# AntreasAntoniou/HowToTrainYourMAMLPytorch

Measured on NVIDIA H100. Metric: meta-tasks/sec (5-way, 5 inner steps, second order), higher is better.
Workload: dtype fp32

## Files before the change

### howtotrainyourmamlpytorch_b200/csrc/engine.cu

```cuda
#include <cstdio>
#include <cstdlib>
#include <cstring>
#include <cmath>
#include <string>
#include <vector>

#include "../../include/maml_b200.h"
#include "common.cuh"
#include "tc_common.cuh"

static thread_local std::string g_err;
static int fail(const std::string& m) { g_err = m; return 1; }

#define CK(call) do { cudaError_t e__ = (call); if (e__ != cudaSuccess) { \
  return fail(std::string(#call) + ": " + cudaGetErrorString(e__)); } } while (0)

static inline long long rup(long long x, long long m) { return (x + m - 1) / m * m; }

struct Profiler {
  struct Rec { int cat; double flops; cudaEvent_t a, b; };
  std::vector<Rec> recs;
  std::vector<cudaEvent_t> pool;
  size_t used = 0;
  cudaEvent_t get() {
// ... 115 lines not shown
static thread_local LaunchContext g_launch_ctx{&g_default_options, false, nullptr, nullptr};
const LaunchContext& launch_ctx() { return g_launch_ctx; }

struct LaunchScope {
  LaunchContext saved;
  explicit LaunchScope(maml_b200_handle* h) : LaunchScope(h, false, nullptr) {}
  LaunchScope(maml_b200_handle* h, cudaStream_t main) : LaunchScope(h, h->pdl, main) {}
  ~LaunchScope() { g_launch_ctx = saved; }
 private:
  LaunchScope(maml_b200_handle* h, bool pdl, cudaStream_t main) : saved(g_launch_ctx) {
    g_launch_ctx = LaunchContext{&h->opt, pdl, main, h->profiling ? &h->prof : nullptr};
  }
};

int num_sms() {
  static int n = 0;
  if (n == 0) {
    int dev = 0;
    if (cudaGetDevice(&dev) != cudaSuccess || cudaDeviceGetAttribute(&n, cudaDevAttrMultiProcessorCount, dev) != cudaSuccess || n <= 0) n = 132;
  }
  return n;
}

extern "C" int maml_b200_abi_version(void) { return MAML_B200_ABI_VERSION; }
extern "C" const char* maml_b200_last_error(void) { return g_err.c_str(); }

static void build_geometry(maml_b200_handle* h) {
  int hh = h->H, ww = h->W, cin = h->C;
  for (int l = 0; l < h->L; ++l) {
    LayerGeom& g = h->geo[l];
    g.h = hh; g.w = ww; g.cin = cin;
    g.gw = ww + 1; g.G = (hh + 1) * (ww + 1);
    g.ph = hh / 2; g.pw = ww / 2;
    if (l < h->L - 1) { g.pgw = g.pw + 1; g.pG = (g.ph + 1) * (g.pw + 1); g.pb = 1; }
    else { g.pgw = g.pw; g.pG = g.ph * g.pw; g.pb = 0; }
    g.guard = g.gw + 2;
    hh = g.ph; ww = g.pw; cin = h->F;
  }
  h->pix = h->geo[h->L - 1].ph * h->geo[h->L - 1].pw;
  h->D = h->pix * h->F;
}

static void build_layout(maml_b200_handle* h) {
  ParamLayout& pl = h->pl;
  memset(&pl, 0, sizeof(pl));
  pl.L = h->L; pl.F = h->F; pl.N = h->N; pl.S = h->S; pl.per_step_bn = h->cfg.per_step_bn; pl.pix = h->pix;
  long long o = 0, m = 0;
  const long long bnsz = (long long)(pl.per_step_bn ? h->S : 1) * h->F;
  for (int l = 0; l < h->L; ++l) {
    pl.cin[l] = h->geo[l].cin;
    const long long wsz = 9LL * pl.cin[l] * h->F;
    pl.w_off[l] = o; o += wsz;
    pl.b_off[l] = o; o += h->F;
    pl.m_w[l] = m; h->seg_off.push_back(m); h->seg_size.push_back(wsz); m += wsz;
    pl.m_b[l] = m; h->seg_off.push_back(m); h->seg_size.push_back(h->F); m += h->F;
    pl.m_beta[l] = m; h->seg_off.push_back(m); h->seg_size.push_back(bnsz); m += bnsz;
    pl.m_gamma[l] = m; h->seg_off.push_back(m); h->seg_size.push_back(bnsz); m += bnsz;
    pl.seg_off[2 * l] = pl.w_off[l]; pl.seg_size[2 * l] = wsz;
    pl.seg_off[2 * l + 1] = pl.b_off[l]; pl.seg_size[2 * l + 1] = h->F;
  }
  pl.fcw_off = o; o += (long long)h->N * h->D;
  pl.fcb_off = o; o += h->N;
  pl.P = o;
  pl.m_fcw = m; h->seg_off.push_back(m); h->seg_size.push_back((long long)h->N * h->D); m += (long long)h->N * h->D;
  pl.m_fcb = m; h->seg_off.push_back(m); h->seg_size.push_back(h->N); m += h->N;
  pl.nseg_inner = 2 * h->L + 2;
  pl.seg_off[2 * h->L] = pl.fcw_off; pl.seg_size[2 * h->L] = (long long)h->N * h->D;
  pl.seg_off[2 * h->L + 1] = pl.fcb_off; pl.seg_size[2 * h->L + 1] = h->N;
  pl.m_lslr = m;
  for (int k = 0; k < pl.nseg_inner; ++k) { h->seg_off.push_back(m); h->seg_size.push_back(h->S + 1); m += h->S + 1; }
  pl.meta_size = m;
  h->Ppad = rup(pl.P, 64);
}

static void plan_chunks(maml_b200_handle* h, int n, ChunkPlan* cp) {
  long long off = 0;
  memset(&cp->pd, 0, sizeof(cp->pd));
  for (int l = 0; l < h->L; ++l) {
    const long long rows = (long long)n * h->geo[l].G;
    int nch, rpc;
    if (l == 0) {
      nch = (int)std::min<long long>(512, std::max<long long>(1, (rows + 63) / 64));
    } else {
      long long want = std::max<long long>(1, num_sms() / (3LL * h->maxT));
      nch = (int)std::min<long long>(std::min<long long>(64, want), std::max<long long>(1, (rows + 15) / 16));
    }
    rpc = (int)rup((rows + nch - 1) / nch, 16);
    nch = (int)((rows + rpc - 1) / rpc);
    cp->rows_per_chunk[l] = rpc; cp->nchunks[l] = nch;
    const long long cs = 9LL * h->geo[l].cin * h->F + h->F;
    cp->pd.off[2 * l] = off; cp->pd.cstride[2 * l] = cs; cp->pd.nchunks[2 * l] = nch;
    cp->pd.off[2 * l + 1] = off + 9LL * h->geo[l].cin * h->F; cp->pd.cstride[2 * l + 1] = cs; cp->pd.nchunks[2 * l + 1] = nch;
    off += cs * nch;
  }
  const int hg = (n + head_rows(n) - 1) / head_rows(n);
  const long long hcs = (long long)h->N * h->D + h->N;
  cp->head_groups = hg;
  cp->pd.off[2 * h->L] = off; cp->pd.cstride[2 * h->L] = hcs; cp->pd.nchunks[2 * h->L] = hg;
  cp->pd.off[2 * h->L + 1] = off + (long long)h->N * h->D; cp->pd.cstride[2 * h->L + 1] = hcs; cp->pd.nchunks[2 * h->L + 1] = hg;
  off += hcs * hg;
  cp->size = rup(off, 64);
  cp->pd.task_stride = cp->size;
}

struct Bump {
  char* base; long long off;
  float* f(long long count) { float* p = base ? (float*)(base + off) : nullptr; off += rup(count * 4, 256); return p; }
  double* d(long long count) { double* p = base ? (double*)(base + off) : nullptr; off += rup(count * 8, 256); return p; }
};

typedef CUresult (*EncodeTiledFn)(CUtensorMap*, CUtensorMapDataType, cuuint32_t, void*, const cuuint64_t*, const cuuint64_t*,
                                  const cuuint32_t*, const cuuint32_t*, CUtensorMapInterleave, CUtensorMapSwizzle,
                                  CUtensorMapL2promotion, CUtensorMapFloatOOBfill);
static EncodeTiledFn get_encode_fn() {
  static EncodeTiledFn fn = nullptr;
  if (!fn) {
    void* p = nullptr;
    cudaDriverEntryPointQueryResult q;
    if (cudaGetDriverEntryPoint("cuTensorMapEncodeTiled", &p, cudaEnableDefault, &q) == cudaSuccess && q == cudaDriverEntryPointSuccess)
      fn = (EncodeTiledFn)p;
  }
  return fn;
}
static int make_map(CUtensorMap* m, const float* base, long long rows, int cols, int box_rows,
                    CUtensorMapSwizzle swz = CU_TENSOR_MAP_SWIZZLE_128B) {
  EncodeTiledFn fn = get_encode_fn();
  if (!fn) return fail("cuTensorMapEncodeTiled entry point not available");
  cuuint64_t gdim[2] = {(cuuint64_t)cols, (cuuint64_t)rows};
  cuuint64_t gstride[1] = {(cuuint64_t)cols * sizeof(float)};
  cuuint32_t box[2] = {32u, (cuuint32_t)box_rows};
  cuuint32_t estr[2] = {1u, 1u};
  CUresult r = fn(m, CU_TENSOR_MAP_DATA_TYPE_FLOAT32, 2, (void*)base, gdim, gstride, box, estr, CU_TENSOR_MAP_INTERLEAVE_NONE,
                  swz, CU_TENSOR_MAP_L2_PROMOTION_L2_128B, CU_TENSOR_MAP_FLOAT_OOB_FILL_NONE);
  if (r != CUDA_SUCCESS) return fail("cuTensorMapEncodeTiled failed with code " + std::to_string((int)r));
  return 0;
}
static int make_pass_maps(maml_b200_handle* h, PassSet& ps, bool has_dz) {
  for (int l = 1; l < h->L; ++l) {
    for (int pl = 0; pl < 2; ++pl) {
      const int rp = tc_conv_rpad(h->geo[l].gw);
      if (make_map(&ps.ain_map[l][pl], ps.ain_base[l] + (pl + 1) * ps.ain_plane[l], ps.ain_plane[l] / h->F, h->F, rp)) return 1;
      if (has_dz && make_map(&ps.dz_map[l][pl], ps.dz_base[l] + (pl + 1) * ps.dz_plane[l], ps.dz_plane[l] / h->F, h->F, rp)) return 1;
    }
  }
  return 0;
}
static int make_all_maps(maml_b200_handle* h) {
  if (!h->use_tc) return 0;
  if (make_pass_maps(h, h->sup, true) || make_pass_maps(h, h->tgt, true) || make_pass_maps(h, h->tan, true)) return 1;
  for (int pl = 0; pl < 4; ++pl) {
    if (make_map(&h->theta_map[pl], h->pack_theta + pl * h->pack_theta_plane, h->pack_theta_plane / h->F, h->F, h->F)) return 1;
    if (make_map(&h->u_map[pl], h->pack_u + pl * h->pack_u_plane, h->pack_u_plane / h->F, h->F, h->F)) return 1;
  }
  if (tc_conv_prepare()) return fail("cudaFuncSetAttribute(max dynamic shared memory) failed for the wgmma conv kernel");
  return 0;
}

static void carve_pass(maml_b200_handle* h, Bump& b, PassSet& ps, int n, int slots, bool need_x, bool need_bwd) {
  ps.n = n; ps.slots = slots;
  const long long T = h->maxT;
  if (need_x) {
    const long long gr = (long long)h->geo[0].guard * h->C;
    const long long body = (long long)n * h->geo[0].G * h->C;
    ps.xg_stride = rup(body + 2 * gr, 64);
    float* p = b.f(ps.xg_stride * T);
    ps.xg = p ? p + gr : nullptr;
  }
  for (int l = 1; l < h->L; ++l) {
    const long long gr = (long long)h->geo[l].guard * h->F;
    const long long body = (long long)n * h->geo[l].G * h->F;
    ps.ain_sz[l] = rup(body + 2 * gr, 192);
    ps.ain_plane[l] = ps.ain_sz[l] * T * slots;
    float* p = b.f(ps.ain_plane[l] * 3);
    ps.ain_base[l] = p;
    ps.ain[l] = p ? p + gr : nullptr;
  }
  ps.ain_sz[h->L] = rup((long long)n * h->D, 64);
  ps.ain[h->L] = b.f(ps.ain_sz[h->L] * T * slots);
  for (int l = 0; l < h->L; ++l) {
    ps.zh_sz[l] = rup((long long)n * h->geo[l].G * h->F, 64);
    ps.zh[l] = b.f(ps.zh_sz[l] * T * slots);
    if (need_bwd) {
      const long long gr = (long long)h->geo[l].guard * h->F;
      ps.dz_sz[l] = rup((long long)n * h->geo[l].G * h->F + 2 * gr, 192);
      ps.dz_plane[l] = ps.dz_sz[l] * T * slots;
      float* p = b.f(ps.dz_plane[l] * 3);
      ps.dz_base[l] = p;
      ps.dz[l] = p ? p + gr : nullptr;
      ps.dp_sz[l] = rup((long long)n * h->geo[l].pG * h->F, 64);
      ps.dp[l] = b.f(ps.dp_sz[l] * T * slots);
    }
  }
}

static void carve(maml_b200_handle* h, Bump& b) {
  const long long T = h->maxT;
  carve_pass(h, b, h->sup, h->n_s, h->S, true, true);
  h->tgt_slots = std::min(h->S, 2);
  carve_pass(h, b, h->tgt, h->n_t, (h->cfg.reserved & 1) ? h->S : h->tgt_slots, true, true);
  carve_pass(h, b, h->tan, h->n_s, 1, false, true);
  carve_pass(h, b, h->tan2, h->n_s, 1, false, true);
  h->theta = b.f((long long)(h->S + 1) * T * h->Ppad);
  h->g = b.f((long long)h->S * T * h->Ppad);
  h->tgrad = b.f((long long)h->S * T * h->Ppad);
  h->tbar = b.f(T * h->Ppad);
  h->u = b.f(T * h->Ppad);
  h->pack_task = (long long)(h->L - 1) * 9 * h->F * h->F;
  h->pack_theta_plane = (long long)(h->S + 1) * T * h->pack_task;
  h->pack_u_plane = T * h->pack_task;
  if (h->use_tc && h->L > 1) {
    h->pack_theta = b.f(4 * h->pack_theta_plane);
    h->pack_u = b.f(4 * h->pack_u_plane);
  }
  h->sup_partial = b.f(T * h->plan_sup.size);
  h->tgt_partial = b.f(T * h->plan_tgt.size * h->tgt_slots);
  h->st_layer_stride = (long long)h->F * 2;
  h->st_pass_stride = (long long)h->L * h->F * 2;
  h->stats_task_stride = (long long)PASS_KINDS * MAML_MAX_STEPS * h->st_pass_stride;
  h->stats_count = h->stats_task_stride * T;
  h->stats = b.d(h->stats_count);
  h->losses = b.f(T * MAML_MAX_STEPS);
  h->correct = b.f(T);
  h->abar = b.d(T * h->pl.nseg_inner * MAML_MAX_STEPS);
  h->decay_dev = b.f(MAML_MAX_STEPS);
  h->zero_labels = (long long*)b.d(std::max(h->n_s, h->n_t));
}

extern "C" int maml_b200_create(const maml_b200_config* cfg, maml_b200_handle** out) {
  if (!cfg || !out) return fail("null argument");
  if (cfg->filters % 16 != 0 || cfg->filters < 16 || cfg->filters > 64) return fail("filters must be a multiple of 16 in [16, 64]");
  if (cfg->num_stages < 1 || cfg->num_stages > MAML_MAX_LAYERS) return fail("num_stages must be in [1, 4]");
  if (cfg->inner_steps < 1 || cfg->inner_steps > MAML_MAX_STEPS) return fail("inner_steps must be in [1, 8]");
  if (cfg->channels < 1 || cfg->channels > 4) return fail("channels must be in [1, 4]");
  if (cfg->max_tasks < 1) return fail("max_tasks must be >= 1");
  if (cfg->n_way < 2 || cfg->n_way > 32) return fail("n_way must be in [2, 32]");
  const int n_s = cfg->n_way * cfg->k_shot, n_t = cfg->n_way * cfg->t_target;
  if (n_s < 1 || n_t < 1 || n_s > 128 || n_t > 128) return fail("N*K and N*T must be in [1, 128]");
  {
    int hh = cfg->height, ww = cfg->width;
    for (int l = 0; l < cfg->num_stages; ++l) { if (hh < 2 || ww < 2) return fail("image too small for num_stages"); hh /= 2; ww /= 2; }
  }
  maml_b200_handle* h = new maml_b200_handle();
  h->cfg = *cfg;
  h->opt = read_options();
  h->L = cfg->num_stages; h->F = cfg->filters; h->N = cfg->n_way; h->S = cfg->inner_steps;
  h->C = cfg->channels; h->H = cfg->height; h->W = cfg->width; h->n_s = n_s; h->n_t = n_t; h->maxT = cfg->max_tasks;
  build_geometry(h);
  build_layout(h);
  h->use_tc = (h->L > 1) && !(cfg->reserved & 2);
  for (int l = 1; l < h->L && h->use_tc; ++l) {
    const int gw = h->geo[l].gw;
    if (tc_conv_rpad(gw) > 256 || tc_conv_ring(h->F, gw, tc_conv_extra_bytes(h->F, 2, true)) < 2) h->use_tc = false;
  }
  plan_chunks(h, h->n_s, &h->plan_sup);
  plan_chunks(h, h->n_t, &h->plan_tgt);
  Bump sz{nullptr, 0};
  carve(h, sz);
  h->ws_bytes = sz.off;
  cudaError_t e = cudaMalloc((void**)&h->ws, (size_t)h->ws_bytes);
  if (e != cudaSuccess) { std::string m = std::string("cudaMalloc workspace (") + std::to_string(h->ws_bytes) + " B): " + cudaGetErrorString(e); delete h; return fail(m); }
  e = cudaMemset(h->ws, 0, (size_t)h->ws_bytes);
  if (e != cudaSuccess) { cudaFree(h->ws); delete h; return fail(std::string("cudaMemset: ") + cudaGetErrorString(e)); }
  Bump as{h->ws, 0};
  carve(h, as);
  if (make_all_maps(h)) { cudaFree(h->ws); delete h; return 1; }
  e = cudaMallocHost((void**)&h->pinned, 16 * 32 * sizeof(float));
  if (e != cudaSuccess) { cudaFree(h->ws); delete h; return fail(std::string("cudaMallocHost: ") + cudaGetErrorString(e)); }
  h->use_graphs = !(cfg->reserved & 4) && !h->opt.no_graph;
  {
    const int l1 = h->L > 1 ? 1 : 0;
    const long long tiles = (((long long)h->n_s * h->geo[l1].G + 127) / 128 + ((long long)h->n_t * h->geo[l1].G + 127) / 128) * h->maxT;
    const bool small = tiles <= num_sms();
    h->pdl = h->opt.pdl >= 0 ? h->opt.pdl != 0 : small;
    h->nb_main = h->opt.tc_nb > 0 ? h->opt.tc_nb : (small ? 8 : 4);
  }
  int prio_lo = 0, prio_hi = 0;
  cudaDeviceGetStreamPriorityRange(&prio_lo, &prio_hi);
  const int p_main = prio_hi, p_tgt = std::min(prio_lo, prio_hi + 1), p_wg = prio_lo;
  bool ok = cudaStreamCreateWithPriority(&h->s_cap, cudaStreamNonBlocking, p_main) == cudaSuccess &&
            cudaStreamCreateWithPriority(&h->s_tgt, cudaStreamNonBlocking, p_tgt) == cudaSuccess &&
            cudaStreamCreateWithPriority(&h->s_tgt2, cudaStreamNonBlocking, p_tgt) == cudaSuccess &&
            cudaStreamCreateWithPriority(&h->s_wg, cudaStreamNonBlocking, p_wg) == cudaSuccess &&
            cudaEventCreateWithFlags(&h->ev_fork, cudaEventDisableTiming) == cudaSuccess &&
            cudaEventCreateWithFlags(&h->ev_wg, cudaEventDisableTiming) == cudaSuccess &&
            cudaEventCreateWithFlags(&h->ev_pack, cudaEventDisableTiming) == cudaSuccess;
  for (int s = 0; ok && s < MAML_MAX_STEPS; ++s) ok = cudaEventCreateWithFlags(&h->ev_tgt[s], cudaEventDisableTiming) == cudaSuccess;
  for (int s = 0; ok && s < 2 * MAML_MAX_LAYERS; ++s) ok = cudaEventCreateWithFlags(&h->ev_pre[s], cudaEventDisableTiming) == cudaSuccess;
  if (!ok) { maml_b200_destroy(h); return fail("stream / event creation failed"); }
  *out = h;
  return 0;
}

static void comm_release(maml_b200_handle* h) {
  for (int p = 0; p < MAML_MAX_RANKS; ++p) if (h->comm_opened[p]) { cudaIpcCloseMemHandle(h->comm_opened[p]); h->comm_opened[p] = nullptr; }
  if (h->comm_block) { cudaFree(h->comm_block); h->comm_block = nullptr; }
  h->comm = CommDev{}; h->comm_connected = false;
}

extern "C" void maml_b200_destroy(maml_b200_handle* h) {
  if (!h) return;
  comm_release(h);
  for (auto& g : h->graphs) if (g.exec) cudaGraphExecDestroy(g.exec);
  if (h->s_cap) cudaStreamDestroy(h->s_cap);
  if (h->s_tgt) cudaStreamDestroy(h->s_tgt);
  if (h->s_tgt2) cudaStreamDestroy(h->s_tgt2);
  if (h->s_wg) cudaStreamDestroy(h->s_wg);
  if (h->ev_fork) cudaEventDestroy(h->ev_fork);
// ... 1085 lines not shown
```

### howtotrainyourmamlpytorch_b200/csrc/kernels_tc.cu

```cuda
#include <cuda.h>
#include <algorithm>
#include <map>
#include <utility>
#include "common.cuh"
#include "tc_common.cuh"

namespace {


__device__ __forceinline__ uint32_t smem_u32(const void* p) { return (uint32_t)__cvta_generic_to_shared(p); }

__device__ __forceinline__ void mbar_init(uint64_t* bar, uint32_t count) {
  asm volatile("mbarrier.init.shared::cta.b64 [%0], %1;" ::"r"(smem_u32(bar)), "r"(count) : "memory");
}
__device__ __forceinline__ void fence_barrier_init() { asm volatile("fence.mbarrier_init.release.cluster;" ::: "memory"); }
__device__ __forceinline__ void mbar_arrive_expect_tx(uint64_t* bar, uint32_t bytes) {
  asm volatile("mbarrier.arrive.expect_tx.shared::cta.b64 _, [%0], %1;" ::"r"(smem_u32(bar)), "r"(bytes) : "memory");
}
__device__ __forceinline__ void mbar_wait(uint64_t* bar, uint32_t parity) {
  const uint32_t addr = smem_u32(bar);
  uint32_t done = 0;
  for (long long spin = 0; spin < (1LL << 26); ++spin) {
    asm volatile("{\n\t.reg .pred p;\n\tmbarrier.try_wait.parity.shared::cta.b64 p, [%1], %2;\n\tselp.u32 %0, 1, 0, p;\n\t}"
                 : "=r"(done) : "r"(addr), "r"(parity) : "memory");
// ... 243 lines not shown
        const int lp = ph - ph_lo;
        ab = lp & 1;
        mbar_wait(&a_full[ab], ((uint32_t)lp >> 1) & 1u);
        if (st == st_lo && threadIdx.x == 0) TC_MARK(2);
        const uint32_t a_hi = smem_u32(smem + (size_t)ab * 2 * abuf) + (uint32_t)(wg * 64 * 128);
        ahd = desc_base + (uint64_t)(a_hi >> 4);
        ald = ahd + (uint64_t)(abuf >> 4);
      }
      mbar_wait(&b_full[stage], bphase);
      if (threadIdx.x == 0) { if (st == st_lo) TC_MARK(3); if (st == st_lo + 9) TC_MARK(4); }
      const int ty = tap / 3;
      const int row_off = a.halo + a.sign * ((ty - 1) * a.gw + (tap - 3 * ty - 1));
      const uint64_t ah0 = ahd + (uint64_t)(row_off * 8);
      const uint64_t al0 = ald + (uint64_t)(row_off * 8);
      const uint64_t bh0 = desc_base + (uint64_t)(smem_u32(bring + (size_t)stage * BSTAGE) >> 4);
      const uint64_t bl0 = bh0 + (uint64_t)(B_BYTES >> 4);
      wgmma_fence();
#pragma unroll
      for (int k = 0; k < 4; ++k) {
        wgmma_tf32<NCOLS>(acc[4], al0 + 2 * k, bh0 + 2 * k);
        wgmma_tf32<NCOLS>(acc[4], ah0 + 2 * k, bl0 + 2 * k);
        wgmma_tf32<NCOLS>(acc[k], ah0 + 2 * k, bh0 + 2 * k);
      }
      wgmma_commit();
      wgmma_wait<1>();
      if (prev_stage >= 0 && lane == 0) {
        mbar_arrive(&b_empty[prev_stage]);
        if (prev_ab >= 0) mbar_arrive(&a_empty[prev_ab]);
      }
      prev_stage = stage;
      prev_ab = (tap == 8 || st == st_hi - 1) ? ab : -1;
      if (++stage == nb) { stage = 0; bphase ^= 1u; }
    }
    wgmma_wait<0>();
#pragma unroll
    for (int q = 0; q < 5; ++q) reg_fence<R>(acc[q]);
    if (threadIdx.x == 0) TC_MARK(5);
    asm volatile("bar.sync 1, 256;" ::: "memory");
    if (threadIdx.x == 0) TC_MARK(6);
    {
      const int rbase = wg * 64 + (warp & 3) * 16 + (lane >> 2);
      const int cq = (lane & 3) * 2;
#pragma unroll
      for (int i = 0; i < NCOLS / 8; ++i) {
#pragma unroll
        for (int hh = 0; hh < 2; ++hh) {
          float o[2];
#pragma unroll
          for (int e = 0; e < 2; ++e) {
            const int x = 4 * i + 2 * hh + e;
            const float big = (acc[0][x] + acc[1][x]) + (acc[2][x] + acc[3][x]);
            o[e] = big + acc[4][x];
          }
          *reinterpret_cast<float2*>(tile + (rbase + 8 * hh) * P4 + 8 * i + cq) = make_float2(o[0], o[1]);
        }
      }
    }
    asm volatile("bar.sync 1, 256;" ::: "memory");
    if (warp < 4) {
      const int r = threadIdx.x;
      const int grow = j0 + r;
      float* trow = tile + r * P4;
      if (nsplit == 1) {
        float* orow = a.out + (long long)task * a.out_stride + (long long)grow * NCOLS;
        const bool want_stats = (a.mode != CONV_PLAIN);
#pragma unroll
        for (int c = 0; c < NCOLS; c += 4) {
          float4 v = *reinterpret_cast<const float4*>(trow + c);
          v.x += s_bias[c]; v.y += s_bias[c + 1]; v.z += s_bias[c + 2]; v.w += s_bias[c + 3];
          if (grow < a.rows) *reinterpret_cast<float4*>(orow + c) = v;
          if (want_stats) *reinterpret_cast<float4*>(trow + c) = v;
        }
      } else {
        cluster_wait();
        const int rows_per = 128 / nsplit, owner = r / rows_per, rloc = r - owner * rows_per;
        const int recv_off = (zrank * rows_per + rloc) * P4;
        const uint32_t push_row = dsmem_addr(smem_u32(recv + recv_off), (uint32_t)owner);
        float* push_local = recv + recv_off;
#pragma unroll
        for (int c = 0; c < NCOLS; c += 4) {
          const float4 v = *reinterpret_cast<const float4*>(trow + c);
          if (owner == zrank) *reinterpret_cast<float4*>(push_local + c) = v;
          else dsmem_st4(push_row + (uint32_t)(c * 4), v);
        }
      }
      if (r == 0) TC_MARK(7);
    }

    int row_lo = 0, row_n = 128;
    const float* sbuf = tile;
    if (nsplit > 1) {
      __syncwarp();
      if (warp >= 4) cluster_wait();
      cluster_sync_all();
      if (threadIdx.x == 0) TC_MARK(10);
      row_n = 128 / nsplit; row_lo = zrank * row_n;
      float* tile2 = reinterpret_cast<float*>(smem + 40 * 1024);
      sbuf = tile2;
      if (warp < 4) {
        const int et = threadIdx.x;
        const float* bias = a.bias ? a.bias + (long long)task * a.bias_stride : nullptr;
        float* outp = a.out + (long long)task * a.out_stride;
        if (nsplit == 2) splitk_reduce<NCOLS, 2>(recv, zrank, et, bias, tile2, outp, j0, a.rows);
        else if (nsplit == 4) splitk_reduce<NCOLS, 4>(recv, zrank, et, bias, tile2, outp, j0, a.rows);
        else splitk_reduce<NCOLS, 8>(recv, zrank, et, bias, tile2, outp, j0, a.rows);
      }
    }

    if (threadIdx.x == 0) TC_MARK(11);
    if (warp < 4) {
      const int et = threadIdx.x;
      const bool want_stats = (a.mode != CONV_PLAIN);
      if (want_stats) {
        asm volatile("bar.sync 2, 128;" ::: "memory");
        constexpr int PARTS = 128 / NCOLS;
        const int col = et % NCOLS, part = et / NCOLS;
        double s1 = 0.0, s2 = 0.0;
        if (part < PARTS) {
          for (int rr = part; rr < row_n; rr += PARTS) {
            if (row_ok[row_lo + rr]) {
              const float v = sbuf[rr * P4 + col];
              if (a.mode == CONV_FWD_STATS) { s1 += (double)v; s2 += (double)v * (double)v; }
              else { s1 += (double)v; s2 += (double)zbuf[rr * P4 + col] * (double)v; }
            }
          }
          if (part < 2) { sred[part][col][0] = s1; sred[part][col][1] = s2; }
        }
        if (PARTS > 2) {
          asm volatile("bar.sync 2, 128;" ::: "memory");
          if (part >= 2 && part < PARTS) { atomicAdd(&sred[part & 1][col][0], s1); atomicAdd(&sred[part & 1][col][1], s2); }
        }
        asm volatile("bar.sync 2, 128;" ::: "memory");
        if (et < NCOLS * 2) {
          const int c = et >> 1, which = et & 1;
          double* stats = a.stats + (long long)task * a.stats_stride;
          atomicAdd(&stats[c * 2 + which], sred[0][c][which] + sred[1][c][which]);
        }
      }
    }
    if (threadIdx.x == 0) TC_MARK(12);
    if (threadIdx.x == 0) TC_MARK(8);
  }
  trace_mark(22 | 0x80, a.tag);
}

template <int NC>
__device__ __forceinline__ void wgmma_tf32_rs(float (&d)[NC / 2], const uint32_t (&a)[4], uint64_t bdesc) {
  if constexpr (NC == 16) wgmma_tf32_rs_n16(d, a, bdesc);
  else if constexpr (NC == 32) wgmma_tf32_rs_n32(d, a, bdesc);
  else if constexpr (NC == 48) wgmma_tf32_rs_n48(d, a, bdesc);
  else wgmma_tf32_rs_n64(d, a, bdesc);
}

template <int NC>
__global__ void __launch_bounds__(128) wgrad_tc_kernel(const WgradArgs a) {
  pdl_prologue(27, a.tag);
  constexpr int R = NC / 2;
  constexpr int BT = NC * 128;
  constexpr int DV = NC / 16;
  extern __shared__ uint8_t smem_raw[];
  uint8_t* smem = reinterpret_cast<uint8_t*>((reinterpret_cast<uintptr_t>(smem_raw) + 1023) & ~(uintptr_t)1023);
  const int task = blockIdx.y;
  const int chunk = blockIdx.x / 9, tap = blockIdx.x - chunk * 9;
  const int ky = tap / 3, kx = tap - 3 * ky;
  const int sh = (ky - 1) * a.gw + (kx - 1);
  const int r_begin = chunk * a.rows_per_chunk;
  const int r_end = min(a.rows, r_begin + a.rows_per_chunk);
  const int guard = a.gw + 2;
  const int KC = a.kc;
  const int tid = threadIdx.x, warp = tid >> 5, lane = tid & 31;
  const int c0 = 16 * warp + (lane >> 2), t4 = lane & 3;
  const int steps = (r_end - r_begin + 31) / 32;
  const int nit = steps * a.nsrc;

  float big[R], small[R], tot[R];
#pragma unroll
  for (int i = 0; i < R; ++i) { big[i] = 0.f; small[i] = 0.f; tot[i] = 0.f; }
  float4 dh[DV], dl[DV];
  auto fetch_d = [&](int it) {
    const int s = it / steps;
    const int r0 = r_begin + (it - s * steps) * 32;
    const float* Dh = a.D[s] + (long long)task * a.d_stride[s] + a.d_plane[s];
    const float* Dl = Dh + a.d_plane[s];
#pragma unroll
    for (int v = 0; v < DV; ++v) {
      const int e = tid + 128 * v, r = e / (NC / 4), f4 = e - r * (NC / 4);
      const int jr = r0 + r;
      const bool ok = jr < r_end;
      dh[v] = ok ? *reinterpret_cast<const float4*>(Dh + (long long)jr * NC + f4 * 4) : make_float4(0.f, 0.f, 0.f, 0.f);
      dl[v] = ok ? *reinterpret_cast<const float4*>(Dl + (long long)jr * NC + f4 * 4) : make_float4(0.f, 0.f, 0.f, 0.f);
    }
  };
  auto drain = [&]() {
    wgmma_wait<0>();
    reg_fence<R>(big);
    reg_fence<R>(small);
#pragma unroll
    for (int i = 0; i < R; ++i) { tot[i] += big[i] + small[i]; big[i] = 0.f; small[i] = 0.f; }
  };

  const uint64_t desc_h = make_desc_sw128(smem_u32(smem)), desc_l = desc_h + (uint64_t)(BT >> 4);
  if (nit > 0) fetch_d(0);
  for (int it = 0; it < nit; ++it) {
    const int s = it / steps;
    const int r0 = r_begin + (it - s * steps) * 32;
#pragma unroll
    for (int v = 0; v < DV; ++v) {
      const int e = tid + 128 * v, r = e / (NC / 4), f4 = e - r * (NC / 4);
      const float hv[4] = {dh[v].x, dh[v].y, dh[v].z, dh[v].w}, lv[4] = {dl[v].x, dl[v].y, dl[v].z, dl[v].w};
#pragma unroll
      for (int q = 0; q < 4; ++q) {
        const int f = f4 * 4 + q;
        const int off = f * 128 + (((r >> 2) ^ (f & 7)) << 4) + (r & 3) * 4;
        *reinterpret_cast<float*>(smem + off) = hv[q];
        *reinterpret_cast<float*>(smem + BT + off) = lv[q];
      }
    }
    asm volatile("fence.proxy.async.shared::cta;" ::: "memory");
    __syncthreads();
    const float* Ah = a.A[s] + (long long)task * a.a_stride[s] + a.a_plane[s];
    const float* Al = Ah + a.a_plane[s];
    uint32_t ah[4][4], al[4][4];
#pragma unroll
    for (int k = 0; k < 4; ++k)
#pragma unroll
      for (int q = 0; q < 4; ++q) {
        const int row = r0 + 8 * k + t4 + ((q & 2) ? 4 : 0);
        const int c = c0 + ((q & 1) ? 8 : 0);
        const int jr = row + sh;
        const bool ok = row < r_end && c < KC && jr >= -guard && jr < a.rows + guard;
        ah[k][q] = ok ? __float_as_uint(Ah[(long long)jr * KC + c]) : 0u;
        al[k][q] = ok ? __float_as_uint(Al[(long long)jr * KC + c]) : 0u;
      }
    const int ks = min(4, (r_end - r0 + 7) >> 3);
#pragma unroll
    for (int k = 0; k < 4; ++k) {
      if (k < ks) {
        wgmma_fence();
        wgmma_tf32_rs<NC>(big, ah[k], desc_h + 2 * k);
        wgmma_tf32_rs<NC>(small, ah[k], desc_l + 2 * k);
        wgmma_tf32_rs<NC>(small, al[k], desc_h + 2 * k);
        wgmma_commit();
      }
    }
    if (it + 1 < nit) fetch_d(it + 1);
    drain();
    __syncthreads();
  }

  float* P = a.partial + (long long)task * a.partial_task_stride + (long long)chunk * a.chunk_stride;
#pragma unroll
  for (int i = 0; i < NC / 8; ++i)
#pragma unroll
    for (int hh = 0; hh < 2; ++hh) {
      const int c = c0 + 8 * hh;
      if (c < KC)
        *reinterpret_cast<float2*>(P + (long long)(tap * KC + c) * NC + 8 * i + 2 * t4) = make_float2(tot[4 * i + 2 * hh], tot[4 * i + 2 * hh + 1]);
    }
  if (tap == 4 && tid < NC) {
    const float* D0 = a.D[0] + (long long)task * a.d_stride[0];
    float bacc = 0.f;
    for (int j = r_begin; j < r_end; ++j) bacc += D0[(long long)j * NC + tid];
    P[(long long)9 * KC * NC + tid] = bacc;
  }
}


}

int tc_read_timeline(long long* out16) { return cudaMemcpyFromSymbol(out16, g_tc_timeline, 16 * sizeof(long long)) == cudaSuccess ? 0 : 1; }

void launch_wgrad_tc(const WgradArgs& a, cudaStream_t st) {
  ProfScope prof_scope__(PROF_WGRAD, a.alg_flops, st);
  dim3 grid(a.nchunks * 9, a.tasks);
  const size_t smem = (size_t)2 * a.ncols * 128 + 1024;
  if (a.ncols == 64) launch_pdl(wgrad_tc_kernel<64>, grid, dim3(128), smem, st, tagged(a));
  else if (a.ncols == 48) launch_pdl(wgrad_tc_kernel<48>, grid, dim3(128), smem, st, tagged(a));
  else if (a.ncols == 32) launch_pdl(wgrad_tc_kernel<32>, grid, dim3(128), smem, st, tagged(a));
  else launch_pdl(wgrad_tc_kernel<16>, grid, dim3(128), smem, st, tagged(a));
  CUDA_CHECK_LAUNCH();
}

int tc_conv_rpad(int gw) { return ((128 + 2 * (gw + 1)) + 7) / 8 * 8; }
int tc_conv_ring(int ncols, int gw, size_t extra) {
  const long long avail = 227LL * 1024 - 4096  - 1024  - 4LL * tc_conv_rpad(gw) * 128 - (long long)extra;
  long long nb = avail / (2LL * ncols * 128);
  if (nb > 8) nb = 8;
  return (int)nb;
}
size_t tc_conv_extra_bytes(int ncols, int S, bool tangent) {
  const size_t row = (size_t)(ncols + 4) * 4;
  return (S > 1 ? 128 * row : 0) + (tangent ? (size_t)(128 / S) * row : 0);
}
static size_t tc_conv_smem_for(int ncols, int gw, int nb) { return (size_t)4 * tc_conv_rpad(gw) * 128 + (size_t)nb * 2 * ncols * 128 + 1024; }

int tc_conv_prepare() {
  const int maxs = 227 * 1024 - 4096;
  cudaError_t e1 = cudaFuncSetAttribute(conv_tc_kernel<64>, cudaFuncAttributeMaxDynamicSharedMemorySize, maxs);
  cudaError_t e2 = cudaFuncSetAttribute(conv_tc_kernel<32>, cudaFuncAttributeMaxDynamicSharedMemorySize, maxs);
  cudaError_t e3 = cudaFuncSetAttribute(conv_tc_kernel<48>, cudaFuncAttributeMaxDynamicSharedMemorySize, maxs);
  cudaError_t e4 = cudaFuncSetAttribute(conv_tc_kernel<16>, cudaFuncAttributeMaxDynamicSharedMemorySize, maxs);
  return (e1 == cudaSuccess && e2 == cudaSuccess && e3 == cudaSuccess && e4 == cudaSuccess) ? 0 : 1;
}

template <int NCOLS>
static int max_clusters(size_t smem, int S) {
  static std::map<std::pair<size_t, int>, int> cache;
  auto it = cache.find({smem, S});
  if (it != cache.end()) return it->second;
  cudaLaunchConfig_t cfg{};
  cfg.gridDim = dim3(1, 1, S); cfg.blockDim = dim3(TC_THREADS); cfg.dynamicSmemBytes = smem;
  cudaLaunchAttribute attr[1];
  attr[0].id = cudaLaunchAttributeClusterDimension;
  attr[0].val.clusterDim.x = 1; attr[0].val.clusterDim.y = 1; attr[0].val.clusterDim.z = S;
  cfg.attrs = attr; cfg.numAttrs = 1;
  int n = 0;
  if (cudaOccupancyMaxActiveClusters(&n, conv_tc_kernel<NCOLS>, &cfg) != cudaSuccess) { cudaGetLastError(); n = 0; }
  cache[{smem, S}] = n;
  return n;
}

template <int NCOLS>
static void launch_conv_tc_n(const TcMaps& maps, const TcConvArgs& a_in, cudaStream_t st) {
  TcConvArgs a = a_in;
  const int tiles = ((a.rows + 127) / 128) * (a.plan_tasks > a.tasks ? a.plan_tasks : a.tasks);
  const int stages = ((a.kc + 31) / 32) * 9;
  const size_t recv_bytes = tc_conv_extra_bytes(NCOLS, 2, false);
  const size_t split_smem = tc_conv_smem_for(NCOLS, a.gw, std::min(a.nb, tc_conv_ring(NCOLS, a.gw, recv_bytes))) + recv_bytes;
  int S = 1;
  for (int cand = launch_ctx().opt->tc_split; cand >= 2; cand >>= 1) {
    if (cand > 8 || stages < 2 * cand) continue;
    if (tiles <= max_clusters<NCOLS>(split_smem, cand)) { S = cand; break; }
  }
  dim3 grid((a.rows + 127) / 128, a.tasks, S);
  const size_t extra = tc_conv_extra_bytes(NCOLS, S, a.mode == CONV_TAN_STATS);
  a.nb = std::min(a.nb, tc_conv_ring(NCOLS, a.gw, extra));
  const size_t smem = tc_conv_smem_for(NCOLS, a.gw, a.nb) + extra;
  if (S == 1) {
    launch_pdl(conv_tc_kernel<NCOLS>, grid, dim3(TC_THREADS), smem, st, maps, tagged(a));
    return;
  }
  cudaLaunchConfig_t cfg{};
  cfg.gridDim = grid; cfg.blockDim = dim3(TC_THREADS); cfg.dynamicSmemBytes = smem; cfg.stream = st;
  cudaLaunchAttribute attr[1];
  attr[0].id = cudaLaunchAttributeClusterDimension;
  attr[0].val.clusterDim.x = 1; attr[0].val.clusterDim.y = 1; attr[0].val.clusterDim.z = S;
  cfg.attrs = attr; cfg.numAttrs = 1;
  cudaLaunchKernelEx(&cfg, conv_tc_kernel<NCOLS>, maps, tagged(a));
}

void launch_conv_tc(const TcMaps& maps, const TcConvArgs& a, cudaStream_t st) {
  ProfScope prof_scope__(PROF_CONV, a.alg_flops, st);
  if (a.ncols == 64) launch_conv_tc_n<64>(maps, a, st);
  else if (a.ncols == 48) launch_conv_tc_n<48>(maps, a, st);
  else if (a.ncols == 32) launch_conv_tc_n<32>(maps, a, st);
  else launch_conv_tc_n<16>(maps, a, st);
  CUDA_CHECK_LAUNCH();
}

__device__ __forceinline__ float tf32_rna(float x) {
  uint32_t r;
  asm("cvt.rna.tf32.f32 %0, %1;" : "=r"(r) : "f"(x));
  return __uint_as_float(r);
}

__global__ void pack_weights_kernel(ParamLayout pl, const float* __restrict__ theta, long long theta_task_stride,
                                    float* __restrict__ pack, long long pack_task_stride, long long plane_stride, int tag) {
  pdl_prologue(21, tag);
  const int task = blockIdx.y;
  const long long per_layer = 9LL * pl.F * pl.F;
  const long long i = (long long)blockIdx.x * blockDim.x + threadIdx.x;
  if (i >= per_layer * (pl.L - 1)) return;
  const int l = 1 + (int)(i / per_layer);
  const long long rel = i - (long long)(l - 1) * per_layer;
  const int f = (int)(rel % pl.F);
  const int c = (int)((rel / pl.F) % pl.F);
  const int tap = (int)(rel / ((long long)pl.F * pl.F));
  const float x = theta[(long long)task * theta_task_stride + pl.w_off[l] + rel];
  const float hi = tf32_rna(x), lo = tf32_rna(x - hi);
  float* p = pack + (long long)task * pack_task_stride + (long long)(l - 1) * per_layer;
  p[rel] = hi;
  p[plane_stride + rel] = lo;
  const long long t = ((long long)tap * pl.F + f) * pl.F + c;
  p[2 * plane_stride + t] = hi;
  p[3 * plane_stride + t] = lo;
}

void launch_pack_weights(const ParamLayout& pl, const float* theta, long long theta_task_stride, float* pack,
                         long long pack_task_stride, long long plane_stride, int tasks, cudaStream_t st) {
  ProfScope prof_scope__(PROF_PARAM, 0.0, st);
  const long long n = 9LL * pl.F * pl.F * (pl.L - 1);
  if (n <= 0) return;
  dim3 grid((unsigned)((n + 255) / 256), tasks);
  launch_pdl(pack_weights_kernel, dim3(grid), dim3(256), (size_t)(0), st, pl, theta, theta_task_stride, pack, pack_task_stride, plane_stride, launch_tag());
  CUDA_CHECK_LAUNCH();
}

MAML_TRACE_SETTER(trace_set_tc)
```

Before: 2197.

## Rewrite wgrad kernel to share D tiles across three kx taps with cp.async pipeline

The weight-gradient kernel now uses one 384-thread CTA per (chunk, ky) row, with three warpgroups covering the three kx taps. Before, there was one 128-thread CTA per tap. The D tile is loaded once per row of taps instead of once per tap. D and A tiles are staged through a 3-slot cp.async/mbarrier pipeline in shared memory, and the transpose into the swizzled wgmma layout overlaps with the wgmma. The bias sum now reads from the staged tile instead of a separate serial loop over global memory. The cost is much larger shared memory, one CTA per SM, and fewer CTAs (grid/3). It also assumes KC == NC when indexing A.

New measurement: 2445, median of 6. +11.3%, better.

```diff
diff --git a/howtotrainyourmamlpytorch_b200/csrc/engine.cu b/howtotrainyourmamlpytorch_b200/csrc/engine.cu
--- a/howtotrainyourmamlpytorch_b200/csrc/engine.cu
+++ b/howtotrainyourmamlpytorch_b200/csrc/engine.cu
@@ -291,7 +291,7 @@
     if (make_map(&h->theta_map[pl], h->pack_theta + pl * h->pack_theta_plane, h->pack_theta_plane / h->F, h->F, h->F)) return 1;
     if (make_map(&h->u_map[pl], h->pack_u + pl * h->pack_u_plane, h->pack_u_plane / h->F, h->F, h->F)) return 1;
   }
-  if (tc_conv_prepare()) return fail("cudaFuncSetAttribute(max dynamic shared memory) failed for the wgmma conv kernel");
+  if (tc_conv_prepare()) return fail("cudaFuncSetAttribute(max dynamic shared memory) failed for the wgmma conv / weight-gradient kernels");
   return 0;
 }
 
diff --git a/howtotrainyourmamlpytorch_b200/csrc/kernels_tc.cu b/howtotrainyourmamlpytorch_b200/csrc/kernels_tc.cu
--- a/howtotrainyourmamlpytorch_b200/csrc/kernels_tc.cu
+++ b/howtotrainyourmamlpytorch_b200/csrc/kernels_tc.cu
@@ -419,117 +419,158 @@
   else wgmma_tf32_rs_n64(d, a, bdesc);
 }
 
+__device__ __forceinline__ void cp_async16(uint32_t dst, const void* src, bool ok) {
+  asm volatile("cp.async.cg.shared.global [%0], [%1], 16, %2;" ::"r"(dst), "l"(src), "r"(ok ? 16 : 0) : "memory");
+}
+__device__ __forceinline__ void cp_async_arrive(uint64_t* bar) {
+  asm volatile("cp.async.mbarrier.arrive.noinc.shared::cta.b64 [%0];" ::"r"(smem_u32(bar)) : "memory");
+}
+
+constexpr int WG_NS = 3;
+constexpr int WG_THREADS = 384;
+
+template <int NC> struct WgSlot {
+  static constexpr int BT = NC * 128;
+  static constexpr int AP = NC + 8;
+  static constexpr int AW = 34 * AP * 4;
+  static constexpr int DW = 32 * NC * 4;
+  static constexpr int A_OFF = 2 * BT, D_OFF = A_OFF + 2 * AW, DF_OFF = D_OFF + 2 * DW;
+  static constexpr int BYTES = (DF_OFF + DW + 1023) / 1024 * 1024;
+};
+template <int NC> constexpr size_t wgrad_tc_smem() { return (size_t)WG_NS * WgSlot<NC>::BYTES + 1024; }
+
 template <int NC>
-__global__ void __launch_bounds__(128) wgrad_tc_kernel(const WgradArgs a) {
+__global__ void __launch_bounds__(WG_THREADS, 1) wgrad_tc_row_kernel(const WgradArgs a) {
   pdl_prologue(27, a.tag);
+  using S = WgSlot<NC>;
   constexpr int R = NC / 2;
-  constexpr int BT = NC * 128;
-  constexpr int DV = NC / 16;
+  constexpr int Q = NC / 4;
   extern __shared__ uint8_t smem_raw[];
   uint8_t* smem = reinterpret_cast<uint8_t*>((reinterpret_cast<uintptr_t>(smem_raw) + 1023) & ~(uintptr_t)1023);
+  __shared__ uint64_t full[WG_NS];
   const int task = blockIdx.y;
-  const int chunk = blockIdx.x / 9, tap = blockIdx.x - chunk * 9;
-  const int ky = tap / 3, kx = tap - 3 * ky;
-  const int sh = (ky - 1) * a.gw + (kx - 1);
+  const int chunk = blockIdx.x / 3, ky = blockIdx.x - chunk * 3;
+  const int sh0 = (ky - 1) * a.gw - 1;
   const int r_begin = chunk * a.rows_per_chunk;
   const int r_end = min(a.rows, r_begin + a.rows_per_chunk);
   const int guard = a.gw + 2;
-  const int KC = a.kc;
+  const int steps = r_end > r_begin ? (r_end - r_begin + 31) / 32 : 0;
+  const int nit = steps * a.nsrc;
+  const bool bias_cta = (ky == 1);
   const int tid = threadIdx.x, warp = tid >> 5, lane = tid & 31;
-  const int c0 = 16 * warp + (lane >> 2), t4 = lane & 3;
-  const int steps = (r_end - r_begin + 31) / 32;
-  const int nit = steps * a.nsrc;
-
-  float big[R], small[R], tot[R];
-#pragma unroll
-  for (int i = 0; i < R; ++i) { big[i] = 0.f; small[i] = 0.f; tot[i] = 0.f; }
-  float4 dh[DV], dl[DV];
-  auto fetch_d = [&](int it) {
+
+  if (tid == 0) {
+    for (int s = 0; s < WG_NS; ++s) mbar_init(&full[s], WG_THREADS);
+    fence_barrier_init();
+  }
+  __syncthreads();
+
+  auto load_stage = [&](int it) {
+    const int slot = it % WG_NS;
     const int s = it / steps;
     const int r0 = r_begin + (it - s * steps) * 32;
-    const float* Dh = a.D[s] + (long long)task * a.d_stride[s] + a.d_plane[s];
+    const float* Ah = a.A[s] + (long long)task * a.a_stride[s] + a.a_plane[s];
+    const float* Al = Ah + a.a_plane[s];
+    const float* Df = a.D[s] + (long long)task * a.d_stride[s];
+    const float* Dh = Df + a.d_plane[s];
     const float* Dl = Dh + a.d_plane[s];
-#pragma unroll
-    for (int v = 0; v < DV; ++v) {
-      const int e = tid + 128 * v, r = e / (NC / 4), f4 = e - r * (NC / 4);
+    const uint32_t base = smem_u32(smem + (size_t)slot * S::BYTES);
+    for (int e = tid; e < 34 * Q; e += WG_THREADS) {
+      const int r = e / Q, c4 = e - r * Q;
+      const int jr = r0 + sh0 + r;
+      const bool ok = jr >= -guard && jr < a.rows + guard;
+      const long long go = ok ? (long long)jr * NC + c4 * 4 : 0;
+      const uint32_t so = (uint32_t)((r * S::AP + c4 * 4) * 4);
+      cp_async16(base + S::A_OFF + so, Ah + go, ok);
+      cp_async16(base + S::A_OFF + S::AW + so, Al + go, ok);
+    }
+    const bool want_f = bias_cta && s == 0;
+    for (int e = tid; e < 32 * Q; e += WG_THREADS) {
+      const int r = e / Q;
       const int jr = r0 + r;
       const bool ok = jr < r_end;
-      dh[v] = ok ? *reinterpret_cast<const float4*>(Dh + (long long)jr * NC + f4 * 4) : make_float4(0.f, 0.f, 0.f, 0.f);
-      dl[v] = ok ? *reinterpret_cast<const float4*>(Dl + (long long)jr * NC + f4 * 4) : make_float4(0.f, 0.f, 0.f, 0.f);
-    }
+      const long long go = ok ? (long long)jr * NC + (e - r * Q) * 4 : 0;
+      cp_async16(base + S::D_OFF + e * 16, Dh + go, ok);
+      cp_async16(base + S::D_OFF + S::DW + e * 16, Dl + go, ok);
+      if (want_f) cp_async16(base + S::DF_OFF + e * 16, Df + go, ok);
+    }
+    cp_async_arrive(&full[slot]);
   };
-  auto drain = [&]() {
+
+  const int kx = warp >> 2;
+  const int c0 = 16 * (warp & 3) + (lane >> 2), t4 = lane & 3;
+  const bool c_ok = c0 < NC;
+  float big[R], small[R], tot[R];
+#pragma unroll
+  for (int i = 0; i < R; ++i) { big[i] = 0.f; small[i] = 0.f; tot[i] = 0.f; }
+  float bacc = 0.f;
+
+  auto transpose = [&](int it) {
+    const int slot = it % WG_NS;
+    uint8_t* sb = smem + (size_t)slot * S::BYTES;
+    mbar_wait(&full[slot], (uint32_t)(it / WG_NS) & 1u);
+    for (int e = tid; e < 2 * 8 * NC; e += WG_THREADS) {
+      const int pl = e / (8 * NC), rem = e - pl * 8 * NC;
+      const int j4 = rem / NC, f = rem - j4 * NC;
+      const float* src = reinterpret_cast<const float*>(sb + S::D_OFF + pl * S::DW) + (4 * j4) * NC + f;
+      const float4 v = make_float4(src[0], src[NC], src[2 * NC], src[3 * NC]);
+      *reinterpret_cast<float4*>(sb + pl * S::BT + f * 128 + ((j4 ^ (f & 7)) << 4)) = v;
+    }
+    if (bias_cta && tid < NC && it < steps) {
+      const float* df = reinterpret_cast<const float*>(sb + S::DF_OFF) + tid;
+#pragma unroll 8
+      for (int r = 0; r < 32; ++r) bacc += df[r * NC];
+    }
+    asm volatile("fence.proxy.async.shared::cta;" ::: "memory");
+  };
+
+  for (int i = 0; i < WG_NS - 1 && i < nit; ++i) load_stage(i);
+  if (nit > 0) transpose(0);
+  for (int it = 0; it < nit; ++it) {
+    const uint8_t* sb = smem + (size_t)(it % WG_NS) * S::BYTES;
+    __syncthreads();
+    if (it + WG_NS - 1 < nit) load_stage(it + WG_NS - 1);
+    const float* wh = reinterpret_cast<const float*>(sb + S::A_OFF) + (kx + t4) * S::AP + c0;
+    const float* wl = wh + S::AW / 4;
+    uint32_t ah[4][4], al[4][4];
+#pragma unroll
+    for (int k = 0; k < 4; ++k)
+#pragma unroll
+      for (int q = 0; q < 4; ++q) {
+        const int o = (8 * k + ((q & 2) ? 4 : 0)) * S::AP + ((q & 1) ? 8 : 0);
+        ah[k][q] = c_ok ? __float_as_uint(wh[o]) : 0u;
+        al[k][q] = c_ok ? __float_as_uint(wl[o]) : 0u;
+      }
+    const uint64_t desc_h = make_desc_sw128(smem_u32(sb)), desc_l = desc_h + (uint64_t)(S::BT >> 4);
+    wgmma_fence();
+#pragma unroll
+    for (int k = 0; k < 4; ++k) {
+      wgmma_tf32_rs<NC>(big, ah[k], desc_h + 2 * k);
+      wgmma_tf32_rs<NC>(small, ah[k], desc_l + 2 * k);
+      wgmma_tf32_rs<NC>(small, al[k], desc_h + 2 * k);
+    }
+    wgmma_commit();
+    if (it + 1 < nit) transpose(it + 1);
     wgmma_wait<0>();
     reg_fence<R>(big);
     reg_fence<R>(small);
 #pragma unroll
     for (int i = 0; i < R; ++i) { tot[i] += big[i] + small[i]; big[i] = 0.f; small[i] = 0.f; }
-  };
-
-  const uint64_t desc_h = make_desc_sw128(smem_u32(smem)), desc_l = desc_h + (uint64_t)(BT >> 4);
-  if (nit > 0) fetch_d(0);
-  for (int it = 0; it < nit; ++it) {
-    const int s = it / steps;
-    const int r0 = r_begin + (it - s * steps) * 32;
-#pragma unroll
-    for (int v = 0; v < DV; ++v) {
-      const int e = tid + 128 * v, r = e / (NC / 4), f4 = e - r * (NC / 4);
-      const float hv[4] = {dh[v].x, dh[v].y, dh[v].z, dh[v].w}, lv[4] = {dl[v].x, dl[v].y, dl[v].z, dl[v].w};
-#pragma unroll
-      for (int q = 0; q < 4; ++q) {
-        const int f = f4 * 4 + q;
-        const int off = f * 128 + (((r >> 2) ^ (f & 7)) << 4) + (r & 3) * 4;
-        *reinterpret_cast<float*>(smem + off) = hv[q];
-        *reinterpret_cast<float*>(smem + BT + off) = lv[q];
-      }
-    }
-    asm volatile("fence.proxy.async.shared::cta;" ::: "memory");
-    __syncthreads();
-    const float* Ah = a.A[s] + (long long)task * a.a_stride[s] + a.a_plane[s];
-    const float* Al = Ah + a.a_plane[s];
-    uint32_t ah[4][4], al[4][4];
-#pragma unroll
-    for (int k = 0; k < 4; ++k)
-#pragma unroll
-      for (int q = 0; q < 4; ++q) {
-        const int row = r0 + 8 * k + t4 + ((q & 2) ? 4 : 0);
-        const int c = c0 + ((q & 1) ? 8 : 0);
-        const int jr = row + sh;
-        const bool ok = row < r_end && c < KC && jr >= -guard && jr < a.rows + guard;
-        ah[k][q] = ok ? __float_as_uint(Ah[(long long)jr * KC + c]) : 0u;
-        al[k][q] = ok ? __float_as_uint(Al[(long long)jr * KC + c]) : 0u;
-      }
-    const int ks = min(4, (r_end - r0 + 7) >> 3);
-#pragma unroll
-    for (int k = 0; k < 4; ++k) {
-      if (k < ks) {
-        wgmma_fence();
-        wgmma_tf32_rs<NC>(big, ah[k], desc_h + 2 * k);
-        wgmma_tf32_rs<NC>(small, ah[k], desc_l + 2 * k);
-        wgmma_tf32_rs<NC>(small, al[k], desc_h + 2 * k);
-        wgmma_commit();
-      }
-    }
-    if (it + 1 < nit) fetch_d(it + 1);
-    drain();
-    __syncthreads();
-  }
-
-  float* P = a.partial + (long long)task * a.partial_task_stride + (long long)chunk * a.chunk_stride;
+    reg_fence<R>(big);
+    reg_fence<R>(small);
+  }
+
+  float* P = a.partial + (long long)task * a.partial_task_stride + (long long)a.chunk_stride * chunk;
+  const int tap = ky * 3 + kx;
 #pragma unroll
   for (int i = 0; i < NC / 8; ++i)
 #pragma unroll
     for (int hh = 0; hh < 2; ++hh) {
       const int c = c0 + 8 * hh;
-      if (c < KC)
-        *reinterpret_cast<float2*>(P + (long long)(tap * KC + c) * NC + 8 * i + 2 * t4) = make_float2(tot[4 * i + 2 * hh], tot[4 * i + 2 * hh + 1]);
-    }
-  if (tap == 4 && tid < NC) {
-    const float* D0 = a.D[0] + (long long)task * a.d_stride[0];
-    float bacc = 0.f;
-    for (int j = r_begin; j < r_end; ++j) bacc += D0[(long long)j * NC + tid];
-    P[(long long)9 * KC * NC + tid] = bacc;
-  }
+      if (c < NC)
+        *reinterpret_cast<float2*>(P + (long long)(tap * NC + c) * NC + 8 * i + 2 * t4) = make_float2(tot[4 * i + 2 * hh], tot[4 * i + 2 * hh + 1]);
+    }
+  if (bias_cta && tid < NC) P[(long long)9 * NC * NC + tid] = bacc;
 }
 
 
@@ -539,12 +580,11 @@
 
 void launch_wgrad_tc(const WgradArgs& a, cudaStream_t st) {
   ProfScope prof_scope__(PROF_WGRAD, a.alg_flops, st);
-  dim3 grid(a.nchunks * 9, a.tasks);
-  const size_t smem = (size_t)2 * a.ncols * 128 + 1024;
-  if (a.ncols == 64) launch_pdl(wgrad_tc_kernel<64>, grid, dim3(128), smem, st, tagged(a));
-  else if (a.ncols == 48) launch_pdl(wgrad_tc_kernel<48>, grid, dim3(128), smem, st, tagged(a));
-  else if (a.ncols == 32) launch_pdl(wgrad_tc_kernel<32>, grid, dim3(128), smem, st, tagged(a));
-  else launch_pdl(wgrad_tc_kernel<16>, grid, dim3(128), smem, st, tagged(a));
+  dim3 grid(a.nchunks * 3, a.tasks);
+  if (a.ncols == 64) launch_pdl(wgrad_tc_row_kernel<64>, grid, dim3(WG_THREADS), wgrad_tc_smem<64>(), st, tagged(a));
+  else if (a.ncols == 48) launch_pdl(wgrad_tc_row_kernel<48>, grid, dim3(WG_THREADS), wgrad_tc_smem<48>(), st, tagged(a));
+  else if (a.ncols == 32) launch_pdl(wgrad_tc_row_kernel<32>, grid, dim3(WG_THREADS), wgrad_tc_smem<32>(), st, tagged(a));
+  else launch_pdl(wgrad_tc_row_kernel<16>, grid, dim3(WG_THREADS), wgrad_tc_smem<16>(), st, tagged(a));
   CUDA_CHECK_LAUNCH();
 }
 
@@ -567,7 +607,12 @@
   cudaError_t e2 = cudaFuncSetAttribute(conv_tc_kernel<32>, cudaFuncAttributeMaxDynamicSharedMemorySize, maxs);
   cudaError_t e3 = cudaFuncSetAttribute(conv_tc_kernel<48>, cudaFuncAttributeMaxDynamicSharedMemorySize, maxs);
   cudaError_t e4 = cudaFuncSetAttribute(conv_tc_kernel<16>, cudaFuncAttributeMaxDynamicSharedMemorySize, maxs);
-  return (e1 == cudaSuccess && e2 == cudaSuccess && e3 == cudaSuccess && e4 == cudaSuccess) ? 0 : 1;
+  cudaError_t w1 = cudaFuncSetAttribute(wgrad_tc_row_kernel<64>, cudaFuncAttributeMaxDynamicSharedMemorySize, (int)wgrad_tc_smem<64>());
+  cudaError_t w2 = cudaFuncSetAttribute(wgrad_tc_row_kernel<48>, cudaFuncAttributeMaxDynamicSharedMemorySize, (int)wgrad_tc_smem<48>());
+  cudaError_t w3 = cudaFuncSetAttribute(wgrad_tc_row_kernel<32>, cudaFuncAttributeMaxDynamicSharedMemorySize, (int)wgrad_tc_smem<32>());
+  cudaError_t w4 = cudaFuncSetAttribute(wgrad_tc_row_kernel<16>, cudaFuncAttributeMaxDynamicSharedMemorySize, (int)wgrad_tc_smem<16>());
+  return (e1 == cudaSuccess && e2 == cudaSuccess && e3 == cudaSuccess && e4 == cudaSuccess && w1 == cudaSuccess &&
+          w2 == cudaSuccess && w3 == cudaSuccess && w4 == cudaSuccess) ? 0 : 1;
 }
 
 template <int NCOLS>
```
